# colmap/glomap

Measured on NVIDIA H100. Metric: observations/sec per BA LM-iteration, higher is better.
Workload: dtype f64

## Files before the change

### glomap_b200/csrc/b200sfm.cu

```cuda
#include "../../include/b200sfm.h"

#include <new>

#include "ba_solver.cuh"
#include "context.cuh"
#include "gp_solver.cuh"
#include "ra_solver.cuh"
#include "track_kernels.cuh"

namespace {

cudaStream_t pool_stream(const b200sfm_ctx* ctx) {
  static const bool dist_pool = !(getenv("B200SFM_ASYNC_ALLOC_DIST") && atoi(getenv("B200SFM_ASYNC_ALLOC_DIST")) == 0);
  return ctx && (ctx->world == 1 || dist_pool) ? ctx->stream : nullptr;
}

template <class F>
int guarded(b200sfm_ctx* ctx, F&& f) {
  b200::AllocScope alloc_scope(pool_stream(ctx));
  try {
    return f();
  } catch (const b200::CudaError& e) {
    if (ctx) ctx->err = "CUDA error: " + e.msg + " (line " + std::to_string(e.line) + ")";
    return B200SFM_ERR_CUDA;
// ... 155 lines not shown
void b200sfm_destroy(b200sfm_ctx* ctx) {
  if (!ctx) return;
  cudaSetDevice(ctx->device);
  if (ctx->comm) nccl_api().CommDestroy(ctx->comm);
  if (ctx->p2p.ready) {
    cudaStreamSynchronize(ctx->stream);
    if (ctx->comm) {
      double* d = nullptr;
      if (cudaMalloc(&d, sizeof(double)) == cudaSuccess) {
        cudaMemsetAsync(d, 0, sizeof(double), ctx->stream);
        nccl_api().AllReduce(d, d, 1, ncclFloat64, ncclSum, ctx->comm, ctx->stream);
        cudaStreamSynchronize(ctx->stream);
        cudaFree(d);
      }
    }
    ctx->p2p.release();
  }
  if (ctx->comm_stream) {
    cudaStreamSynchronize(ctx->comm_stream);
    cudaStreamDestroy(ctx->comm_stream);
    cudaEventDestroy(ctx->ev_half);
    cudaEventDestroy(ctx->ev_comm);
  }
  if (ctx->stream) {
    cudaStreamSynchronize(ctx->stream);
    cudaStreamDestroy(ctx->stream);
  }
  if (b200::async_alloc_enabled()) {
    cudaMemPool_t pool;
    if (cudaDeviceGetDefaultMemPool(&pool, ctx->device) == cudaSuccess) cudaMemPoolTrimTo(pool, 0);
    cudaGetLastError();
  }
  if (ctx->h_scal) cudaFreeHost(ctx->h_scal);
  delete ctx;
}

const char* b200sfm_last_error(const b200sfm_ctx* ctx) { return ctx ? ctx->err.c_str() : "null context"; }
int b200sfm_rank(const b200sfm_ctx* ctx) { return ctx ? ctx->rank : -1; }
int b200sfm_world_size(const b200sfm_ctx* ctx) { return ctx ? ctx->world : -1; }
void* b200sfm_cuda_stream(const b200sfm_ctx* ctx) { return ctx ? (void*)ctx->stream : nullptr; }
int64_t b200sfm_kernel_launches(const b200sfm_ctx* ctx) { return ctx ? ctx->launches : 0; }

void b200sfm_ba_default_opts(b200sfm_ba_opts* o) {
  if (!o) return;
  std::memset(o, 0, sizeof(*o));
  o->optimize_rig_poses = 0;
// ... 645 lines not shown
```

### glomap_b200/csrc/ba_kernels_v2.cuh

```cuda
#pragma once
#include "ba_kernels.cuh"
#include "pcg.cuh"

namespace b200 {

struct BAViewV2 {
  const double* Ap;
  double* z4;
  const double* pts4;
  double* Ufk = nullptr;
  const IntrVarRec* ivar = nullptr;
  int C = 0;
};

template <int NK>
__device__ __forceinline__ void obs_intr_rows(const ObsCore& o, const double* __restrict__ ir, const IntrVarRec& iv,
                                              const double Jp[6], double Jk[2][NK > 0 ? NK : 1],
                                              double B[NK > 0 ? 3 * NK : 1]) {
#pragma unroll
  for (int j = 0; j < NK; ++j) {
    double jx = 0.0, jy = 0.0;
    if (j < iv.mb) intr_param_jac(ir, iv.pidx[j], o.uv[0], o.uv[1], 1.0, jx, jy);
    if (!o.valid) jx = jy = 0.0;
    Jk[0][j] = jx;
// ... 473 lines not shown
  a3 = block_sum(a3, scratch);
  if (threadIdx.x == 0) {
    double* o = out + 4 * (size_t)blockIdx.x;
    o[0] = a0; o[1] = a1; o[2] = a2; o[3] = a3;
  }
}

__global__ void ba2_point_rhs_z(BAView v, BAViewV2 v2) {
  const int p = blockIdx.x * blockDim.x + threadIdx.x;
  if (p >= v.P) return;
  double vi[6], g[3], z[3];
#pragma unroll
  for (int k = 0; k < 6; ++k) vi[k] = v.Vinv[6 * (size_t)p + k];
#pragma unroll
  for (int k = 0; k < 3; ++k) g[k] = v.gp[3 * (size_t)p + k];
  sym3_mul(vi, g, z);
  const bool pvalid = (int)(v.pt_begin[p + 1] - v.pt_begin[p]) >= v.min_views;
  *reinterpret_cast<double4*>(v2.z4 + 4 * (size_t)p) = pvalid ? make_double4(z[0], z[1], z[2], 0.0) : make_double4(0, 0, 0, 0);
}

template <int NK>
__global__ void __launch_bounds__(128, B200_PB_MIN_CTAS) ba2_pass_b(BAView v, BAViewV2 v2, const double* __restrict__ cam_rec,
                                                 const double* __restrict__ intr_rec, double huber_a,
                                                 double* __restrict__ y, const PcgCtl* __restrict__ ctl, int seg_lo,
                                                 int seg_hi) {
  if (ctl && ctl->done) return;
  const int warp = seg_lo + ((blockIdx.x * blockDim.x + threadIdx.x) >> 5);
  const int lane = threadIdx.x & 31;
  if (warp >= seg_hi) return;
  const int cam = v.seg_cam[warp];
  const int b = v.seg_begin[warp], e = v.seg_end[warp];
  const double4 q4c = ld_rec32(cam_rec + (size_t)cam * kCamRec);
  const double4 t4c = ld_rec32(cam_rec + (size_t)cam * kCamRec + 4);
  const int blk = v.seg_intr[warp];
  const double* irc = intr_rec + (size_t)blk * kIntrRec;
  const double* src = sensor_of_seg(v, warp);
  constexpr int NKK = NK > 0 ? NK : 1;
  IntrVarRec iv{};
  if (NK > 0) iv = v2.ivar[blk];
  double acc[6] = {0, 0, 0, 0, 0, 0};
  double accK[NKK];
#pragma unroll
  for (int k = 0; k < NKK; ++k) accK[k] = 0.0;
  const uint64_t keep = l2_policy_evict_last();
  int i = b + lane;
  int pt_nxt = 0;
  double4 X = make_double4(0, 0, 0, 0), z = X;
  double2 xy = make_double2(0, 0);
  if (i < e) {
    const int pt0 = ld_stream(v.pt_c + i);
    if (i + 32 < e) pt_nxt = ld_stream(v.pt_c + i + 32);
    X = ld_rec32(v2.pts4 + 4 * (size_t)pt0);
    z = ld_keep4(v2.z4 + 4 * (size_t)pt0, keep);
    xy = ld_stream(v.xy_c + i);
  }
  for (; i < e; i += 32) {
    double4 Xn = X, zn = z;
    double2 xyn = xy;
    int pt_nn = 0;
    if (i + 32 < e) {
      Xn = ld_rec32(v2.pts4 + 4 * (size_t)pt_nxt);
      zn = ld_keep4(v2.z4 + 4 * (size_t)pt_nxt, keep);
      xyn = ld_stream(v.xy_c + i + 32);
    }
    if (i + 64 < e) pt_nn = ld_stream(v.pt_c + i + 64);
    ObsCore o;
    obs_core(q4c, t4c, irc, src, X.x, X.y, X.z, xy, huber_a, o);
    double Jp[6], a[6], bo[3];
    obs_point_blocks(o, Jp, a, bo);
    const double w0 = a[0] * z.x + a[1] * z.y + a[2] * z.z;
    const double w1 = a[1] * z.x + a[3] * z.y + a[4] * z.z;
    const double w2 = a[2] * z.x + a[4] * z.y + a[5] * z.z;
    acc[0] += 2.0 * (X.y * w2 - X.z * w1);
    acc[1] += 2.0 * (X.z * w0 - X.x * w2);
    acc[2] += 2.0 * (X.x * w1 - X.y * w0);
    acc[3] += w0;
    acc[4] += w1;
    acc[5] += w2;
    if (NK > 0) {
      double Jk[2][NKK], Bo[3 * NKK];
      obs_intr_rows<NK>(o, irc, iv, Jp, Jk, Bo);
#pragma unroll
      for (int k = 0; k < NK; ++k) accK[k] += Bo[3 * k] * z.x + Bo[3 * k + 1] * z.y + Bo[3 * k + 2] * z.z;
    }
    X = Xn; z = zn; xy = xyn; pt_nxt = pt_nn;
  }
#pragma unroll
  for (int k = 0; k < 6; ++k) acc[k] = warp_sum(acc[k]);
  if (lane < 6) {
    const int mask = (int)(__double_as_longlong(t4c.w) & 0xff);
    const double q[4] = {q4c.x, q4c.y, q4c.z, q4c.w};
    double R[9];
    quat_to_R(q, R);
    const int bl = lane / 3, r = lane % 3;
    const bool fixed = bl == 0 ? (mask & 1) : (mask & 2);
    const double s = R[3 * r] * acc[3 * bl] + R[3 * r + 1] * acc[3 * bl + 1] + R[3 * r + 2] * acc[3 * bl + 2];
    if (!fixed && s != 0.0) atomicAdd(&y[(size_t)cam * 6 + lane], -s);
  }
  if (NK > 0) {
    const size_t kb = (size_t)(v2.C + blk);
#pragma unroll
    for (int k = 0; k < NK; ++k) {
      const double sk = warp_sum(accK[k]);
      if (lane == 0 && sk != 0.0) atomicAdd(&y[kb * 6 + k], -sk);
    }
  }
}

__global__ void ba2k_pack_xk(int C, const double* __restrict__ cam_rec, const double* __restrict__ x, double* __restrict__ xp,
                             const PcgCtl* __restrict__ ctl) {
  if (ctl && ctl->done) return;
  const int c = blockIdx.x * blockDim.x + threadIdx.x;
  if (c >= C) return;
  const int blk = (int)(__double_as_longlong(cam_rec[(size_t)c * kCamRec + 7]) >> 8);
  xp[(size_t)c * kXqStride + 6] = x[(size_t)(C + blk) * 6];
  xp[(size_t)c * kXqStride + 7] = x[(size_t)(C + blk) * 6 + 1];
}

template <int NK>
__global__ void __launch_bounds__(256) ba2k_cross(int C, int K, const double* __restrict__ cam_rec, const double* __restrict__ Ufk,
                                                  const double* __restrict__ x, double* __restrict__ y,
                                                  const PcgCtl* __restrict__ ctl) {
  constexpr int kBins = 256;
  __shared__ double bins[kBins * NK];
  if (ctl && ctl->done) return;
  const bool use_bins = K <= kBins;
  if (use_bins) {
// ... 42 lines not shown
```

### glomap_b200/csrc/ba_kernels_v3.cuh

```cuda
#pragma once
#include "ba_kernels_v2.cuh"

namespace b200 {

constexpr int kEllWindow = 1024;
constexpr int kEllThreads = 128;

struct EllView {
  int n_groups;
  const int* row0;
  const int* pt;
  const int* len;
  const int* cam;
  const double2* xy;
  const unsigned short* sensor;
  double* A;
  double* B = nullptr;
};

template <class Sort>
__global__ void __launch_bounds__(kEllWindow) ell_sort_window(int P, int min_views, const unsigned* __restrict__ pt_begin,
                                                              int* __restrict__ ell_pt, int* __restrict__ ell_len,
                                                              int* __restrict__ ell_slot, int* __restrict__ group_rows) {
  __shared__ typename Sort::TempStorage tmp;
// ... 241 lines not shown
  if (threadIdx.x == 0) part_cost[blockIdx.x] = cost;
}

__global__ void __launch_bounds__(1024) ba3_reduce_partials(int n, const double* __restrict__ part_a,
                                                           const double* __restrict__ part_b, double* __restrict__ out_sum,
                                                           double* __restrict__ out_max) {
  __shared__ double scratch[32];
  double s = 0.0, m = 0.0;
  for (int i = threadIdx.x; i < n; i += blockDim.x) {
    s += part_a[i];
    if (part_b) m = fmax(m, part_b[i]);
  }
  s = block_sum(s, scratch);
  if (threadIdx.x == 0) *out_sum = s;
  if (part_b) {
    m = block_max(m, scratch);
    if (threadIdx.x == 0) *out_max = m;
  }
}

template <int MODE, int NK>
__global__ void __launch_bounds__(kEllThreads, MODE == 0 ? B200_EA_MIN_CTAS : B200_EA2_MIN_CTAS) ba3_pass_a(
    BAView v, EllView ell, BAViewV2 v2, const double* __restrict__ xp, const double* __restrict__ points,
    double* __restrict__ points_new, double radius, double* __restrict__ bscal, const PcgCtl* __restrict__ ctl) {
  __shared__ double scratch[32];
  if (ctl && ctl->done) return;
  const int slot = blockIdx.x * kEllThreads + threadIdx.x;
  const int lane = threadIdx.x & 31;
  const int g = slot >> 5;
  double b0 = 0, b1 = 0, b2 = 0, b3 = 0;
  if (g < ell.n_groups) {
    const int pt = ell.pt[slot];
    const int mylen = ell.len[slot];
    const int r0 = ell.row0[g], nrow = ell.row0[g + 1] - r0;
    double X0 = 0, X1 = 0, X2 = 0;
    if (pt >= 0) {
      X0 = points[3 * (size_t)pt]; X1 = points[3 * (size_t)pt + 1]; X2 = points[3 * (size_t)pt + 2];
    }
    double s0 = 0, s1 = 0, s2 = 0;
#pragma unroll 4
    for (int j = 0; j < nrow; ++j) {
      if (j >= mylen) continue;
      const size_t idx = ((size_t)r0 + j) * 32 + lane;
      const int cam = ld_stream(ell.cam + idx);
      const double* row = ell.A + ((size_t)r0 + j) * (6 * 32) + lane;
      const double a0 = ld_stream(row), a1 = ld_stream(row + 32), a2 = ld_stream(row + 64);
      const double a3 = ld_stream(row + 96), a4 = ld_stream(row + 128), a5 = ld_stream(row + 160);
      double xr0, xr1, xr2, xt0;
      ld_nc_256(xp + (size_t)cam * kXqStride, xr0, xr1, xr2, xt0);
      double4 xt;
      if (NK > 0) {
        xt = ld_rec32(xp + (size_t)cam * kXqStride + 4);
      } else {
        const double2 xt12 = __ldg(reinterpret_cast<const double2*>(xp + (size_t)cam * kXqStride + 4));
// ... 71 lines not shown
```

### glomap_b200/csrc/ba_solver.cuh

```cuda
#pragma once
#include <cub/cub.cuh>

#include <algorithm>
#include <climits>
#include <cmath>
#include <cstdlib>
#include <vector>

#include "../../include/b200sfm_testing.h"
#include "ba_kernels.cuh"
#include "ba_kernels_v2.cuh"
#include "ba_kernels_v3.cuh"
#include "ba_kernels_ext.cuh"
#include "filter_kernels.cuh"
#include "processor_kernels.cuh"
#include "context.cuh"
#include "pcg.cuh"

namespace b200 {

constexpr double kSliceL2Share = 1.0 / 6.0;

__global__ void k_expand_obs_pt(int P, const unsigned* __restrict__ pt_begin, int* __restrict__ obs_pt) {
  const int p = blockIdx.x * blockDim.x + threadIdx.x;
// ... 79 lines not shown
  if (n > 0) {
    const double inv = 1.0 / n;
    for (int k = 0; k < 4; ++k) q[4 * c + k] *= inv;
  }
}
__global__ void k_rhs(int n, const double* __restrict__ gc, const double* __restrict__ y, double* __restrict__ b) {
  const int i = blockIdx.x * blockDim.x + threadIdx.x;
  if (i < n) b[i] = -(gc[i] + (y ? y[i] : 0.0));
}

}

struct b200sfm_ba_problem {
  using BAView = b200::BAView;
  template <class T>
  using DevBuf = b200::DevBuf<T>;

  b200sfm_ctx* ctx = nullptr;
  int C = 0, P = 0, K = 0;
  long long N = 0;
  int Nv = 0, n_tiles = 0, n_segs = 0, min_views = 3;
  int seg_mid = 0;
  int n_slices = 1, slice_pts = 0;
  long long n_obs_used = 0;

  DevBuf<int> obs_cam, obs_pt, tile_pt_begin, camord_obs, pt_c, seg_cam, seg_begin, seg_end, cam_intr, intr_model;
  int S = 0;
  DevBuf<unsigned short> obs_sensor;
  DevBuf<int> seg_sensor, seg_intr, sensor_intr;
  DevBuf<double> sensor_rec;
  DevBuf<double2> obs_xy, xy_c;
  DevBuf<int4> tile_desc;
  DevBuf<unsigned> pt_begin;
  DevBuf<unsigned char> cam_mask_base, cam_mask;
  DevBuf<double> blk_used;
  DevBuf<double> quat[2], trans[2], points[2], intr, intr_cand, quat_saved, trans_saved, points_saved, intr_saved;
  int CB = 0, nbk = 0;
  bool ext = false, ext_k = false, ext_s = false;
  std::vector<int> h_intr_model;
  std::vector<b200::IntrVarRec> h_ivar;
  DevBuf<b200::IntrVarRec> ivar;
  std::vector<unsigned char> h_sensor_var;
  DevBuf<unsigned char> sensor_var;
  DevBuf<double> sens_q[2], sens_t[2], sens_q_saved, sens_t_saved;
  b200::ExtView ext_view() {
    b200::ExtView e;
// ... 165 lines not shown
                obs_cam.p, S > 0 ? obs_sensor.p : nullptr, obs_pt.p, pt_begin.p, keys.p, vals.p, cam_count.p, bad.p);
    int end_bit = 1;
    while ((1ll << end_bit) <= n_buckets) ++end_bit;
    size_t tmp_bytes = 0;
    cub::DeviceRadixSort::SortPairs(nullptr, tmp_bytes, keys.p, keys_out.p, vals.p, camord_obs.p, (int)N, 0, end_bit, s);
    size_t scan_bytes = 0;
    cub::DeviceScan::ExclusiveSum(nullptr, scan_bytes, cam_count.p, cam_begin.p, n_buckets + 1, s);
    DevBuf<unsigned char> tmp;
    tmp.alloc(std::max(tmp_bytes, scan_bytes) + 16);
    size_t tb = tmp.bytes();
    cub::DeviceRadixSort::SortPairs(tmp.p, tb, keys.p, keys_out.p, vals.p, camord_obs.p, (int)N, 0, end_bit, s);
    ctx->launches += 8;
    tb = tmp.bytes();
    cub::DeviceScan::ExclusiveSum(tmp.p, tb, cam_count.p, cam_begin.p, n_buckets + 1, s);
    B200_LAUNCH(ctx, k_seg_counts, cdiv(n_buckets, 256), 256, 0, n_buckets, cam_count.p, seg_count.p);
    blk_used.alloc(CB);
    blk_used.zero(s);
    B200_LAUNCH(ctx, k_block_used, cdiv(VC, 256), 256, 0, VC, n_groups, smul, C, K, cam_count.p, cam_intr.p,
                S > 0 ? sensor_intr.p : nullptr, blk_used.p);
    ctx->allreduce_sum(blk_used.p, CB);
    tb = tmp.bytes();
    cub::DeviceScan::ExclusiveSum(tmp.p, tb, seg_count.p, seg_off.p, n_buckets + 1, s);
    ctx->launches += 4;
    int h_tot[4];
    B200_CUDA_OK(cudaMemcpyAsync(&h_tot[0], cam_begin.p + n_buckets, sizeof(int), cudaMemcpyDeviceToHost, s));
    B200_CUDA_OK(cudaMemcpyAsync(&h_tot[1], seg_off.p + n_buckets, sizeof(int), cudaMemcpyDeviceToHost, s));
    B200_CUDA_OK(cudaMemcpyAsync(&h_tot[2], bad.p, sizeof(int), cudaMemcpyDeviceToHost, s));
    B200_CUDA_OK(cudaMemcpyAsync(&h_tot[3], seg_off.p + (size_t)n_slices * VC, sizeof(int), cudaMemcpyDeviceToHost, s));
    B200_CUDA_OK(cudaStreamSynchronize(s));
    if (h_tot[2]) throw InvalidInput{"obs_cam out of range [0, C)"};
    Nv = h_tot[0];
    n_segs = h_tot[1];
    seg_mid = h_tot[3];
    seg_cam.alloc(std::max(n_segs, 1)); seg_begin.alloc(std::max(n_segs, 1)); seg_end.alloc(std::max(n_segs, 1));
    seg_sensor.alloc(std::max(n_segs, 1)); seg_intr.alloc(std::max(n_segs, 1));
    pt_c.alloc(std::max(Nv, 1)); xy_c.alloc(std::max(Nv, 1));
    B200_LAUNCH(ctx, k_fill_segs, cdiv(n_buckets, 256), 256, 0, n_buckets, VC, smul, cam_begin.p, seg_off.p, cam_intr.p,
                S > 0 ? sensor_intr.p : nullptr, seg_cam.p, seg_sensor.p, seg_intr.p, seg_begin.p, seg_end.p);
    if (Nv > 0)
      B200_LAUNCH(ctx, k_gather_camorder, cdiv(Nv, 256), 256, 0, Nv, camord_obs.p, obs_pt.p, obs_xy.p, pt_c.p, xy_c.p);

    {
      using Sort = cub::BlockRadixSort<unsigned, kEllWindow, 1, int>;
      const int n_win = cdiv(P, kEllWindow);
      ell_groups = n_win * (kEllWindow / 32);
      ell_ctas = cdiv((long long)ell_groups * 32, kEllThreads);
      ell_pt.alloc((size_t)ell_groups * 32); ell_len.alloc((size_t)ell_groups * 32); ell_slot.alloc(P);
      ell_row0.alloc((size_t)ell_groups + 1);
      DevBuf<int> grows;
      grows.alloc((size_t)ell_groups + 1);
      grows.zero(s);
      B200_LAUNCH(ctx, (ell_sort_window<Sort>), n_win, kEllWindow, 0, P, min_views, pt_begin.p, ell_pt.p, ell_len.p, ell_slot.p, grows.p);
      size_t need = 0;
      cub::DeviceScan::ExclusiveSum(nullptr, need, grows.p, ell_row0.p, ell_groups + 1, s);
      DevBuf<unsigned char> tmp3;
      tmp3.alloc(need + 16);
// ... 324 lines not shown
    ExtView ex = ext_view();
    const int sgrid = cdiv((long long)n_segs * 32, 128);
    if (x && points_var) {
#define B200_EXT_A(WK, WS)                                                                                              \
  B200_LAUNCH(ctx, (bax_pass_a<0, WK, WS>), ell_ctas, kEllThreads, 0, v, ell_view(), ex, view2(), cam_rec.p, intr_rec.p, x, \
              points[cur].p, nullptr, huber_a, radius, nullptr, ctl)
      if (ext_k && ext_s) B200_EXT_A(true, true);
      else if (ext_k) B200_EXT_A(true, false);
      else if (ext_s) B200_EXT_A(false, true);
      else B200_EXT_A(false, false);
#undef B200_EXT_A
    }
    if (n_segs > 0) {
#define B200_EXT_B(WK, WS)                                                                                              \
  B200_LAUNCH(ctx, (bax_pass_b<WK, WS>), sgrid, 128, 0, v, ex, view2(), cam_rec.p, intr_rec.p, points[cur].p, x, huber_a, y, ctl)
      if (ext_k && ext_s) B200_EXT_B(true, true);
      else if (ext_k) B200_EXT_B(true, false);
      else if (ext_s) B200_EXT_B(false, true);
      else B200_EXT_B(false, false);
#undef B200_EXT_B
    }
  }

  void launch_pass_b(const b200::BAView& v, double huber_a, double* y, const b200::PcgCtl* ctl, int seg_lo = 0,
                     int seg_hi = -1) {
    using namespace b200;
    if (seg_hi < 0) seg_hi = n_segs;
    if (seg_hi <= seg_lo) return;
    const int grid = cdiv((long long)(seg_hi - seg_lo) * 32, 128);
#define B200_PASS_B(NKV) \
  B200_LAUNCH(ctx, ba2_pass_b<NKV>, grid, 128, 0, v, view2(), cam_rec.p, intr_rec.p, huber_a, y, ctl, seg_lo, seg_hi)
    if (kfast && nk == 2) B200_PASS_B(2);
    else if (kfast) B200_PASS_B(1);
    else B200_PASS_B(0);
#undef B200_PASS_B
  }
  void launch_pass_a0(const b200::BAView& v, double radius, const b200::PcgCtl* ctl) {
    using namespace b200;
    if (kfast && nk == 2)
      B200_LAUNCH(ctx, (ba3_pass_a<0, 2>), ell_ctas, kEllThreads, 0, v, ell_view(), view2(), xq.p, points[cur].p, nullptr, radius, nullptr, ctl);
    else if (kfast)
      B200_LAUNCH(ctx, (ba3_pass_a<0, 1>), ell_ctas, kEllThreads, 0, v, ell_view(), view2(), xq.p, points[cur].p, nullptr, radius, nullptr, ctl);
    else
      B200_LAUNCH(ctx, (ba3_pass_a<0, 0>), ell_ctas, kEllThreads, 0, v, ell_view(), view2(), xq.p, points[cur].p, nullptr, radius, nullptr, ctl);
  }
  void launch_cross(const double* x, double* y, const b200::PcgCtl* ctl) {
    using namespace b200;
    if (nk == 2) B200_LAUNCH(ctx, ba2k_cross<2>, cdiv(C, 256), 256, 0, C, K, cam_rec.p, Ufk.p, x, y, ctl);
    else B200_LAUNCH(ctx, ba2k_cross<1>, cdiv(C, 256), 256, 0, C, K, cam_rec.p, Ufk.p, x, y, ctl);
  }

  bool matrix_free() const { return ext && !kfast; }
  bool schur_jacobi_on(const b200sfm_ba_opts& o, bool points_var) const {
    return points_var && o.preconditioner == 1 && !matrix_free();
  }

  void matvec(const double* x, double* y, const b200sfm_ba_opts& o, double radius, bool points_var, bool split_ar,
              bool profile, const b200::PcgCtl* ctl) {
    using namespace b200;
    cudaStream_t s = ctx->stream;
    BAView v = view();
    const int nB6 = nbk * 6;
    cudaEvent_t e0 = nullptr, e1 = nullptr;
    if (profile) {
      e0 = timer_mv.next();
      e1 = timer_mv.next();
      B200_CUDA_OK(cudaEventRecord(e0, s));
    }
    if (matrix_free()) {
      ext_matvec(x, y, o.thres_loss_function, radius, points_var, ctl);
    } else if (kfast && !points_var) {
      launch_cross(x, y, ctl);
    } else if (use_v2) {
      if (use_ell)
        launch_pass_a0(v, radius, ctl);
      else
        B200_LAUNCH(ctx, ba2_pass_a<0>, n_tiles, kTile, smem_k3v2, v, view2(), xq.p, points[cur].p, nullptr, radius, nullptr, ctl);
      if (kfast) launch_cross(x, y, ctl);
      if (split_ar) {
        launch_pass_b(v, o.thres_loss_function, y, ctl, 0, seg_mid);
        B200_CUDA_OK(cudaEventRecord(ctx->ev_half, s));
        B200_CUDA_OK(cudaStreamWaitEvent(ctx->comm_stream, ctx->ev_half, 0));
        ctx->allreduce_sum_on(ctx->comm_stream, y, (size_t)(C / 2) * 6);
        B200_CUDA_OK(cudaEventRecord(ctx->ev_comm, ctx->comm_stream));
        launch_pass_b(v, o.thres_loss_function, y, ctl, seg_mid, n_segs);
      } else if (n_segs > 0) {
        launch_pass_b(v, o.thres_loss_function, y, ctl);
      }
    } else {
      B200_LAUNCH(ctx, ba_schur_pass<0>, n_tiles, kTile, smem_k3, v, x, y, nullptr, nullptr, radius, nullptr, nullptr,
                  nullptr, 0, ctl);
    }
    if (profile) B200_CUDA_OK(cudaEventRecord(e1, s));
    if (split_ar) {
      ctx->allreduce_sum(y + (size_t)(C / 2) * 6, nB6 - (size_t)(C / 2) * 6);
      B200_CUDA_OK(cudaStreamWaitEvent(s, ctx->ev_comm, 0));
    } else {
      ctx->allreduce_sum(y, nB6);
    }
  }

  StepResult compute_step(const b200sfm_ba_opts& o, double radius, bool points_var, bool set_jscale_p, bool profile) {
    using namespace b200;
    cudaStream_t s = ctx->stream;
    BAView v = view();
    const int nB6 = nbk * 6;
    if (points_var) B200_LAUNCH(ctx, ba_damp_points, cdiv(P, 256), 256, 0, P, V.p, jscale_p.p, set_jscale_p ? 1 : 0, radius, Vinv.p);
    B200_LAUNCH(ctx, ba_damp_cams, cdiv(nB6, 256), 256, 0, nbk, U(), jscale_c.p, radius, Dc.p);
    const bool recomp = matrix_free();
    const bool schur_jacobi = schur_jacobi_on(o, points_var);
    double* yrhs = Sd.p + (size_t)CB * 21;
    Sd.zero(s);
    if (schur_jacobi && n_segs > 0) {
      if (use_v2)
        B200_LAUNCH(ctx, ba2_schur_diag, cdiv((long long)n_segs * 32, 128), 128, 0, v, view2(), cam_rec.p, intr_rec.p,
                    o.thres_loss_function);
      else B200_LAUNCH(ctx, ba_schur_diag, cdiv((long long)n_segs * 32, 128), 128, 0, v);
    }
    if (points_var) {
      if (use_v2) {
        B200_LAUNCH(ctx, ba2_point_rhs_z, cdiv(P, 256), 256, 0, v, view2());
        if (recomp) ext_matvec(nullptr, yrhs, o.thres_loss_function, radius, true, nullptr);
        else if (n_segs > 0) launch_pass_b(v, o.thres_loss_function, yrhs, nullptr);
      } else {
        B200_LAUNCH(ctx, ba_schur_pass<1>, n_tiles, kTile, smem_k3, v, nullptr, yrhs, nullptr, nullptr, radius, nullptr);
      }
    } else if (recomp) {
      z4.zero(s);
    }
    if (schur_jacobi || points_var) ctx->allreduce_sum(Sd.p, (size_t)CB * 27);
    B200_LAUNCH(ctx, ba_build_precond, cdiv(nbk, 128), 128, 0, nbk, U(), Dc.p, schur_jacobi ? Sd.p : nullptr, Minv.p);
    B200_LAUNCH(ctx, k_rhs, cdiv(nB6, 256), 256, 0, nB6, gc(), points_var ? yrhs : nullptr, bvec.p);
    const int max_it = std::max(1, o.pcg_max_iterations);
    const int nblk = cdiv(nbk, kPcgThreads);
    ctx->pcgh.ensure(max_it, (size_t)nblk * 3, ctx->world);
    double* part_pq = ctx->pcgh.d_part;
    double* part_rz = ctx->pcgh.d_part + nblk;
    double* part_rr = ctx->pcgh.d_part + 2 * (size_t)nblk;
    PcgCtl* ctl = ctx->pcgh.d_ctl;
    StepResult res;
    const size_t mv_ev0 = timer_mv.used;
    const bool has_mv = points_var || ext;
    const bool split_ar = ctx->world > 1 && use_v2 && !recomp && points_var && C >= 64 &&
                          (getenv("B200SFM_SPLIT_AR") && atoi(getenv("B200SFM_SPLIT_AR")) == 1);
    if (split_ar) ctx->ensure_comm_stream();
    const bool pack_dir = points_var && use_v2 && !recomp;
// ... 32 lines not shown
      B200_CUDA_OK(cudaMemcpyAsync(intr_cand.p, intr.p, intr.bytes(), cudaMemcpyDeviceToDevice, s));
      if (S > 0) {
        B200_CUDA_OK(cudaMemcpyAsync(sens_q[nxt].p, sens_q[cur].p, sens_q[cur].bytes(), cudaMemcpyDeviceToDevice, s));
        B200_CUDA_OK(cudaMemcpyAsync(sens_t[nxt].p, sens_t[cur].p, sens_t[cur].bytes(), cudaMemcpyDeviceToDevice, s));
      }
    }
    if (points_var && use_v2) {
      const int nrow_part = use_ell ? ell_ctas : n_tiles;
      if (recomp) {
        ExtView ex = ext_view();
#define B200_EXT_A2(WK, WS)                                                                                                  \
  B200_LAUNCH(ctx, (bax_pass_a<2, WK, WS>), ell_ctas, kEllThreads, 0, v, ell_view(), ex, view2(), cam_rec.p, intr_rec.p, px.p, \
              points[cur].p, points[nxt].p, o.thres_loss_function, radius, bpart.p, nullptr)
        if (ext_k && ext_s) B200_EXT_A2(true, true);
        else if (ext_k) B200_EXT_A2(true, false);
        else if (ext_s) B200_EXT_A2(false, true);
        else B200_EXT_A2(false, false);
#undef B200_EXT_A2
      } else {
        B200_LAUNCH(ctx, ba2_pack_x, cdiv(C, 256), 256, 0, C, px.p, cam_rec.p, xq.p);
        if (kfast) B200_LAUNCH(ctx, ba2k_pack_xk, cdiv(C, 256), 256, 0, C, cam_rec.p, px.p, xq.p, nullptr);
        if (use_ell && kfast && nk == 2)
          B200_LAUNCH(ctx, (ba3_pass_a<2, 2>), ell_ctas, kEllThreads, 0, v, ell_view(), view2(), xq.p, points[cur].p, points[nxt].p, radius,
                      bpart.p, nullptr);
        else if (use_ell && kfast)
          B200_LAUNCH(ctx, (ba3_pass_a<2, 1>), ell_ctas, kEllThreads, 0, v, ell_view(), view2(), xq.p, points[cur].p, points[nxt].p, radius,
                      bpart.p, nullptr);
        else if (use_ell)
          B200_LAUNCH(ctx, (ba3_pass_a<2, 0>), ell_ctas, kEllThreads, 0, v, ell_view(), view2(), xq.p, points[cur].p, points[nxt].p, radius,
                      bpart.p, nullptr);
        else
          B200_LAUNCH(ctx, ba2_pass_a<2>, n_tiles, kTile, smem_k3v2, v, view2(), xq.p, points[cur].p, points[nxt].p, radius, bpart.p, nullptr);
      }
      const int nb = std::min(cdiv(nrow_part, 256), 296);
      B200_LAUNCH(ctx, ba2_sum4_stage1, nb, 256, 0, nrow_part, bpart.p, bpart2.p);
      B200_LAUNCH(ctx, ba_colsum, 4, 256, 0, nb, 4, bpart2.p, scal.p + 2);
    } else if (points_var) {
      B200_LAUNCH(ctx, ba_schur_pass<2>, n_tiles, kTile, smem_k3, v, px.p, nullptr, points[cur].p, points[nxt].p, radius,
                  scal.p + 2);
    } else {
      B200_CUDA_OK(cudaMemcpyAsync(points[nxt].p, points[cur].p, points[cur].bytes(), cudaMemcpyDeviceToDevice, s));
    }
    B200_LAUNCH(ctx, ba_update_cams, cdiv(C, 128), 128, 0, C, quat[cur].p, trans[cur].p, px.p, gc(), pr.p, Dc.p, jscale_c.p,
                blk_used.p, cam_mask.p, quat[nxt].p, trans[nxt].p, scal.p + 8);
    build_records(nxt);
    launch_cost(nxt, o.thres_loss_function);
    ctx->allreduce_sum(scal.p + 2, 11);
    B200_CUDA_OK(cudaMemcpyAsync(ctx->h_scal, scal.p, 16 * sizeof(double), cudaMemcpyDeviceToHost, s));
    B200_CUDA_OK(cudaStreamSynchronize(s));
    double* h = ctx->h_scal;
    for (int k = 8; k <= 12; ++k) h[k] /= (double)ctx->world;
    const double g_dot_d = h[8] + h[2];
    const double dDd = h[10] + h[3];
// ... 225 lines not shown
```

### glomap_b200/csrc/context.cuh

```cuda
#pragma once
#include <dlfcn.h>
#include <nccl.h>

#include <cstring>
#include <string>
#include <vector>

#include "../../include/b200sfm.h"
#include "common.cuh"
#include "p2p_allreduce.cuh"
#include "pcg.cuh"

struct NcclApi {
  void* lib = nullptr;
  ncclResult_t (*GetUniqueId)(ncclUniqueId*) = nullptr;
  ncclResult_t (*CommInitRank)(ncclComm_t*, int, ncclUniqueId, int) = nullptr;
  ncclResult_t (*CommDestroy)(ncclComm_t) = nullptr;
  ncclResult_t (*CommAbort)(ncclComm_t) = nullptr;
  ncclResult_t (*AllReduce)(const void*, void*, size_t, ncclDataType_t, ncclRedOp_t, ncclComm_t, cudaStream_t) = nullptr;
  const char* (*GetErrorString)(ncclResult_t) = nullptr;
  bool load(std::string& err) {
    if (lib) return true;
    lib = dlopen("libnccl.so.2", RTLD_NOW | RTLD_GLOBAL);
    if (!lib) lib = dlopen("libnccl.so", RTLD_NOW | RTLD_GLOBAL);
// ... 41 lines not shown
  void allreduce_sum(double* buf, size_t n) {
    if (world > 1 && p2p.ready && n > 0 && n <= p2p.cap && (reinterpret_cast<uintptr_t>(buf) & 15) == 0) {
      p2p.launch(stream, buf, n);
      ++p2p_calls;
      ++launches;
      return;
    }
    allreduce_sum_on(stream, buf, n);
  }
  void allreduce_sum_on(cudaStream_t st, double* buf, size_t n) {
    if (world == 1 || n == 0) return;
    if (!comm) throw NcclError{"communicator was aborted after an earlier failure"};
    ncclResult_t r = nccl_api().AllReduce(buf, buf, n, ncclFloat64, ncclSum, comm, st);
    if (r != ncclSuccess) throw NcclError{std::string("ncclAllReduce(sum): ") + nccl_api().GetErrorString(r)};
  }
  cudaStream_t comm_stream = nullptr;
  cudaEvent_t ev_half = nullptr, ev_comm = nullptr;
  void ensure_comm_stream() {
    if (comm_stream) return;
    B200_CUDA_OK(cudaStreamCreateWithFlags(&comm_stream, cudaStreamNonBlocking));
    B200_CUDA_OK(cudaEventCreateWithFlags(&ev_half, cudaEventDisableTiming));
    B200_CUDA_OK(cudaEventCreateWithFlags(&ev_comm, cudaEventDisableTiming));
  }
  void allreduce_max(double* buf, size_t n) {
    if (world == 1 || n == 0) return;
    if (!comm) throw NcclError{"communicator was aborted after an earlier failure"};
    ncclResult_t r = nccl_api().AllReduce(buf, buf, n, ncclFloat64, ncclMax, comm, stream);
    if (r != ncclSuccess) throw NcclError{std::string("ncclAllReduce(max): ") + nccl_api().GetErrorString(r)};
  }
};

namespace b200 {

inline cudaStream_t& alloc_stream() {
  static thread_local cudaStream_t s = nullptr;
  return s;
}
struct AllocScope {
  cudaStream_t prev;
  explicit AllocScope(cudaStream_t s) : prev(alloc_stream()) { alloc_stream() = s; }
  ~AllocScope() { alloc_stream() = prev; }
};
inline bool async_alloc_enabled() {
  static const bool on = !(getenv("B200SFM_ASYNC_ALLOC") && atoi(getenv("B200SFM_ASYNC_ALLOC")) == 0);
  return on;
}
// ... 58 lines not shown
  a.accessPolicyWindow.num_bytes = 0;
  cudaStreamSetAttribute(s, cudaStreamAttributeAccessPolicyWindow, &a);
  cudaCtxResetPersistingL2Cache();
  cudaGetLastError();
}

struct EventTimer {
  std::vector<cudaEvent_t> ev;
  size_t used = 0;
  ~EventTimer() {
    for (auto e : ev) cudaEventDestroy(e);
  }
  cudaEvent_t next() {
    if (used == ev.size()) {
      cudaEvent_t e;
      B200_CUDA_OK(cudaEventCreate(&e));
      ev.push_back(e);
    }
    return ev[used++];
  }
  void reset() { used = 0; }
};

#define B200_LAUNCH(ctx, kernel, grid, block, smem, ...)                       \
  do {                                                                         \
    kernel<<<(grid), (block), (smem), (ctx)->stream>>>(__VA_ARGS__);           \
    ++(ctx)->launches;                                                         \
  } while (0)

inline int cdiv(long long a, long long b) { return (int)((a + b - 1) / b); }

}
```

### profiles/kernel_times.py

```python
#!/usr/bin/env python
import argparse
import collections
import os
import sys

ROOT = os.path.dirname(os.path.dirname(os.path.abspath(__file__)))
sys.path.insert(0, ROOT)


def main():
    ap = argparse.ArgumentParser()
    ap.add_argument("--workload", default="config4")
    ap.add_argument("--optimize-intrinsics", type=int, default=0)
    ap.add_argument("--solves", type=int, default=2)
    ap.add_argument("--top", type=int, default=14)
    args = ap.parse_args()
    import torch
    from bench import WORKLOADS
    from glomap_b200 import estimators as E, synthetic as S

    C, P, L, chunk = WORKLOADS[args.workload]
    sc = S.make_scene(C, P, L, seed=1, pixel_sigma=0.5, chunk=chunk, point_range=(0, P))
    init = S.perturb_scene(sc, chunk=chunk, point_offset=0)
    mask = E.first_frame_mask(C)
    torch.cuda.set_device(0)
    ctx = E.Context(0, 0, 1, None)
    opts = E.BundleAdjusterOptions(optimize_intrinsics=bool(args.optimize_intrinsics))
    opts.solver_options.max_num_iterations = 20
    opts.solver_options.pcg_rel_tolerance = 0.05
    opts.solver_options.pcg_max_iterations = 200
    torch.cuda.synchronize()
    free0 = torch.cuda.mem_get_info()[0]
    prob = E.BAProblem(ctx, sc, 3, mask)
    prob.set_state(init.intr_params, init.quat, init.trans, init.points)
    prob.save_state()
    prob.solve(opts)
    torch.cuda.synchronize()
    free1 = torch.cuda.mem_get_info()[0]
    its = []
    with torch.profiler.profile(activities=[torch.profiler.ProfilerActivity.CUDA]) as prof:
        for _ in range(args.solves):
            prob.restore_state()
            st = prob.solve(opts).as_dict()
            its.append((st["iterations"], st["pcg_iterations"]))
        torch.cuda.synchronize()
    agg = collections.defaultdict(lambda: [0, 0.0])
    for ev in prof.events():
        if ev.device_type == torch.autograd.DeviceType.CUDA and ev.name and not ev.name.startswith("Memcpy") \
                and not ev.name.startswith("Memset"):
            name = ev.name.split("(")[0].replace("void ", "").replace("b200::", "")
            agg[name][0] += 1
            agg[name][1] += ev.device_time_total
    tot = sum(v[1] for v in agg.values())
    print(f"{args.workload} optimize_intrinsics={args.optimize_intrinsics} env="
          f"{ {k: v for k, v in os.environ.items() if k.startswith('B200SFM_')} } LM/PCG per solve {its}")
    print(f"device memory held by the resident problem after one solve: {(free0 - free1) / 1e9:.3f} GB")
    print("| kernel | launches | total ms | avg us |\n|---|---|---|---|")
    for k, (n, us) in sorted(agg.items(), key=lambda kv: -kv[1][1])[:args.top]:
        print(f"| `{k}` | {n} | {us / 1e3:.3f} | {us / n:.1f} |")
    print(f"total kernel time {tot / 1e3 / args.solves:.2f} ms per solve\n")
    prob.free()
    ctx.close()


if __name__ == "__main__":
    main()
```

Measured before the change: 1.155 billion.

## Pipeline Schur matvec by point slice, overlapping pass A and pass B on two streams

Splits the PCG mat-vec into per-point-slice chunks. Pass A runs on the main stream for each slice, and the matching pass B camera segments run on a high-priority second stream, gated by per-slice events, so the two passes overlap instead of running back to back. Both kernels become grid-stride loops over segment ranges with capped grid sizes, and the setup code copies per-slice segment offsets to the host. This adds more launches, event traffic and an extra stream, and it relies on the segment ordering matching the point slices.

```diff
diff --git a/glomap_b200/csrc/b200sfm.cu b/glomap_b200/csrc/b200sfm.cu
--- a/glomap_b200/csrc/b200sfm.cu
+++ b/glomap_b200/csrc/b200sfm.cu
@@ -201,6 +201,11 @@
     cudaEventDestroy(ctx->ev_half);
     cudaEventDestroy(ctx->ev_comm);
   }
+  if (ctx->mv_stream) {
+    cudaStreamSynchronize(ctx->mv_stream);
+    cudaStreamDestroy(ctx->mv_stream);
+  }
+  for (cudaEvent_t e : ctx->mv_ev) cudaEventDestroy(e);
   if (ctx->stream) {
     cudaStreamSynchronize(ctx->stream);
     cudaStreamDestroy(ctx->stream);
diff --git a/glomap_b200/csrc/ba_kernels_v2.cuh b/glomap_b200/csrc/ba_kernels_v2.cuh
--- a/glomap_b200/csrc/ba_kernels_v2.cuh
+++ b/glomap_b200/csrc/ba_kernels_v2.cuh
@@ -519,87 +519,89 @@
 template <int NK>
 __global__ void __launch_bounds__(128, B200_PB_MIN_CTAS) ba2_pass_b(BAView v, BAViewV2 v2, const double* __restrict__ cam_rec,
                                                  const double* __restrict__ intr_rec, double huber_a,
-                                                 double* __restrict__ y, const PcgCtl* __restrict__ ctl, int seg_lo,
-                                                 int seg_hi) {
+                                                 double* __restrict__ y, const PcgCtl* __restrict__ ctl, int lo0,
+                                                 int hi0, int lo1, int hi1) {
   if (ctl && ctl->done) return;
-  const int warp = seg_lo + ((blockIdx.x * blockDim.x + threadIdx.x) >> 5);
   const int lane = threadIdx.x & 31;
-  if (warp >= seg_hi) return;
-  const int cam = v.seg_cam[warp];
-  const int b = v.seg_begin[warp], e = v.seg_end[warp];
-  const double4 q4c = ld_rec32(cam_rec + (size_t)cam * kCamRec);
-  const double4 t4c = ld_rec32(cam_rec + (size_t)cam * kCamRec + 4);
-  const int blk = v.seg_intr[warp];
-  const double* irc = intr_rec + (size_t)blk * kIntrRec;
-  const double* src = sensor_of_seg(v, warp);
-  constexpr int NKK = NK > 0 ? NK : 1;
-  IntrVarRec iv{};
-  if (NK > 0) iv = v2.ivar[blk];
-  double acc[6] = {0, 0, 0, 0, 0, 0};
-  double accK[NKK];
-#pragma unroll
-  for (int k = 0; k < NKK; ++k) accK[k] = 0.0;
-  const uint64_t keep = l2_policy_evict_last();
-  int i = b + lane;
-  int pt_nxt = 0;
-  double4 X = make_double4(0, 0, 0, 0), z = X;
-  double2 xy = make_double2(0, 0);
-  if (i < e) {
-    const int pt0 = ld_stream(v.pt_c + i);
-    if (i + 32 < e) pt_nxt = ld_stream(v.pt_c + i + 32);
-    X = ld_rec32(v2.pts4 + 4 * (size_t)pt0);
-    z = ld_keep4(v2.z4 + 4 * (size_t)pt0, keep);
-    xy = ld_stream(v.xy_c + i);
-  }
-  for (; i < e; i += 32) {
-    double4 Xn = X, zn = z;
-    double2 xyn = xy;
-    int pt_nn = 0;
-    if (i + 32 < e) {
-      Xn = ld_rec32(v2.pts4 + 4 * (size_t)pt_nxt);
-      zn = ld_keep4(v2.z4 + 4 * (size_t)pt_nxt, keep);
-      xyn = ld_stream(v.xy_c + i + 32);
-    }
-    if (i + 64 < e) pt_nn = ld_stream(v.pt_c + i + 64);
-    ObsCore o;
-    obs_core(q4c, t4c, irc, src, X.x, X.y, X.z, xy, huber_a, o);
-    double Jp[6], a[6], bo[3];
-    obs_point_blocks(o, Jp, a, bo);
-    const double w0 = a[0] * z.x + a[1] * z.y + a[2] * z.z;
-    const double w1 = a[1] * z.x + a[3] * z.y + a[4] * z.z;
-    const double w2 = a[2] * z.x + a[4] * z.y + a[5] * z.z;
-    acc[0] += 2.0 * (X.y * w2 - X.z * w1);
-    acc[1] += 2.0 * (X.z * w0 - X.x * w2);
-    acc[2] += 2.0 * (X.x * w1 - X.y * w0);
-    acc[3] += w0;
-    acc[4] += w1;
-    acc[5] += w2;
+  const int n0 = hi0 - lo0, n = n0 + (hi1 - lo1);
+  for (int w = (blockIdx.x * blockDim.x + threadIdx.x) >> 5; w < n; w += (gridDim.x * blockDim.x) >> 5) {
+    const int warp = w < n0 ? lo0 + w : lo1 + (w - n0);
+    const int cam = v.seg_cam[warp];
+    const int b = v.seg_begin[warp], e = v.seg_end[warp];
+    const double4 q4c = ld_rec32(cam_rec + (size_t)cam * kCamRec);
+    const double4 t4c = ld_rec32(cam_rec + (size_t)cam * kCamRec + 4);
+    const int blk = v.seg_intr[warp];
+    const double* irc = intr_rec + (size_t)blk * kIntrRec;
+    const double* src = sensor_of_seg(v, warp);
+    constexpr int NKK = NK > 0 ? NK : 1;
+    IntrVarRec iv{};
+    if (NK > 0) iv = v2.ivar[blk];
+    double acc[6] = {0, 0, 0, 0, 0, 0};
+    double accK[NKK];
+  #pragma unroll
+    for (int k = 0; k < NKK; ++k) accK[k] = 0.0;
+    const uint64_t keep = l2_policy_evict_last();
+    int i = b + lane;
+    int pt_nxt = 0;
+    double4 X = make_double4(0, 0, 0, 0), z = X;
+    double2 xy = make_double2(0, 0);
+    if (i < e) {
+      const int pt0 = ld_stream(v.pt_c + i);
+      if (i + 32 < e) pt_nxt = ld_stream(v.pt_c + i + 32);
+      X = ld_rec32(v2.pts4 + 4 * (size_t)pt0);
+      z = ld_keep4(v2.z4 + 4 * (size_t)pt0, keep);
+      xy = ld_stream(v.xy_c + i);
+    }
+    for (; i < e; i += 32) {
+      double4 Xn = X, zn = z;
+      double2 xyn = xy;
+      int pt_nn = 0;
+      if (i + 32 < e) {
+        Xn = ld_rec32(v2.pts4 + 4 * (size_t)pt_nxt);
+        zn = ld_keep4(v2.z4 + 4 * (size_t)pt_nxt, keep);
+        xyn = ld_stream(v.xy_c + i + 32);
+      }
+      if (i + 64 < e) pt_nn = ld_stream(v.pt_c + i + 64);
+      ObsCore o;
+      obs_core(q4c, t4c, irc, src, X.x, X.y, X.z, xy, huber_a, o);
+      double Jp[6], a[6], bo[3];
+      obs_point_blocks(o, Jp, a, bo);
+      const double w0 = a[0] * z.x + a[1] * z.y + a[2] * z.z;
+      const double w1 = a[1] * z.x + a[3] * z.y + a[4] * z.z;
+      const double w2 = a[2] * z.x + a[4] * z.y + a[5] * z.z;
+      acc[0] += 2.0 * (X.y * w2 - X.z * w1);
+      acc[1] += 2.0 * (X.z * w0 - X.x * w2);
+      acc[2] += 2.0 * (X.x * w1 - X.y * w0);
+      acc[3] += w0;
+      acc[4] += w1;
+      acc[5] += w2;
+      if (NK > 0) {
+        double Jk[2][NKK], Bo[3 * NKK];
+        obs_intr_rows<NK>(o, irc, iv, Jp, Jk, Bo);
+  #pragma unroll
+        for (int k = 0; k < NK; ++k) accK[k] += Bo[3 * k] * z.x + Bo[3 * k + 1] * z.y + Bo[3 * k + 2] * z.z;
+      }
+      X = Xn; z = zn; xy = xyn; pt_nxt = pt_nn;
+    }
+  #pragma unroll
+    for (int k = 0; k < 6; ++k) acc[k] = warp_sum(acc[k]);
+    if (lane < 6) {
+      const int mask = (int)(__double_as_longlong(t4c.w) & 0xff);
+      const double q[4] = {q4c.x, q4c.y, q4c.z, q4c.w};
+      double R[9];
+      quat_to_R(q, R);
+      const int bl = lane / 3, r = lane % 3;
+      const bool fixed = bl == 0 ? (mask & 1) : (mask & 2);
+      const double s = R[3 * r] * acc[3 * bl] + R[3 * r + 1] * acc[3 * bl + 1] + R[3 * r + 2] * acc[3 * bl + 2];
+      if (!fixed && s != 0.0) atomicAdd(&y[(size_t)cam * 6 + lane], -s);
+    }
     if (NK > 0) {
-      double Jk[2][NKK], Bo[3 * NKK];
-      obs_intr_rows<NK>(o, irc, iv, Jp, Jk, Bo);
-#pragma unroll
-      for (int k = 0; k < NK; ++k) accK[k] += Bo[3 * k] * z.x + Bo[3 * k + 1] * z.y + Bo[3 * k + 2] * z.z;
-    }
-    X = Xn; z = zn; xy = xyn; pt_nxt = pt_nn;
-  }
-#pragma unroll
-  for (int k = 0; k < 6; ++k) acc[k] = warp_sum(acc[k]);
-  if (lane < 6) {
-    const int mask = (int)(__double_as_longlong(t4c.w) & 0xff);
-    const double q[4] = {q4c.x, q4c.y, q4c.z, q4c.w};
-    double R[9];
-    quat_to_R(q, R);
-    const int bl = lane / 3, r = lane % 3;
-    const bool fixed = bl == 0 ? (mask & 1) : (mask & 2);
-    const double s = R[3 * r] * acc[3 * bl] + R[3 * r + 1] * acc[3 * bl + 1] + R[3 * r + 2] * acc[3 * bl + 2];
-    if (!fixed && s != 0.0) atomicAdd(&y[(size_t)cam * 6 + lane], -s);
-  }
-  if (NK > 0) {
-    const size_t kb = (size_t)(v2.C + blk);
-#pragma unroll
-    for (int k = 0; k < NK; ++k) {
-      const double sk = warp_sum(accK[k]);
-      if (lane == 0 && sk != 0.0) atomicAdd(&y[kb * 6 + k], -sk);
+      const size_t kb = (size_t)(v2.C + blk);
+  #pragma unroll
+      for (int k = 0; k < NK; ++k) {
+        const double sk = warp_sum(accK[k]);
+        if (lane == 0 && sk != 0.0) atomicAdd(&y[kb * 6 + k], -sk);
+      }
     }
   }
 }
diff --git a/glomap_b200/csrc/ba_kernels_v3.cuh b/glomap_b200/csrc/ba_kernels_v3.cuh
--- a/glomap_b200/csrc/ba_kernels_v3.cuh
+++ b/glomap_b200/csrc/ba_kernels_v3.cuh
@@ -287,14 +287,14 @@
 template <int MODE, int NK>
 __global__ void __launch_bounds__(kEllThreads, MODE == 0 ? B200_EA_MIN_CTAS : B200_EA2_MIN_CTAS) ba3_pass_a(
     BAView v, EllView ell, BAViewV2 v2, const double* __restrict__ xp, const double* __restrict__ points,
-    double* __restrict__ points_new, double radius, double* __restrict__ bscal, const PcgCtl* __restrict__ ctl) {
+    double* __restrict__ points_new, double radius, double* __restrict__ bscal, const PcgCtl* __restrict__ ctl,
+    int g_lo, int g_hi) {
   __shared__ double scratch[32];
   if (ctl && ctl->done) return;
-  const int slot = blockIdx.x * kEllThreads + threadIdx.x;
   const int lane = threadIdx.x & 31;
-  const int g = slot >> 5;
   double b0 = 0, b1 = 0, b2 = 0, b3 = 0;
-  if (g < ell.n_groups) {
+  for (int g = g_lo + ((blockIdx.x * kEllThreads + threadIdx.x) >> 5); g < g_hi; g += gridDim.x * (kEllThreads / 32)) {
+    const int slot = g * 32 + lane;
     const int pt = ell.pt[slot];
     const int mylen = ell.len[slot];
     const int r0 = ell.row0[g], nrow = ell.row0[g + 1] - r0;
diff --git a/glomap_b200/csrc/ba_solver.cuh b/glomap_b200/csrc/ba_solver.cuh
--- a/glomap_b200/csrc/ba_solver.cuh
+++ b/glomap_b200/csrc/ba_solver.cuh
@@ -125,6 +125,7 @@
   int Nv = 0, n_tiles = 0, n_segs = 0, min_views = 3;
   int seg_mid = 0;
   int n_slices = 1, slice_pts = 0;
+  std::vector<int> slice_seg;
   long long n_obs_used = 0;
 
   DevBuf<int> obs_cam, obs_pt, tile_pt_begin, camord_obs, pt_c, seg_cam, seg_begin, seg_end, cam_intr, intr_model;
@@ -336,16 +337,17 @@
     tb = tmp.bytes();
     cub::DeviceScan::ExclusiveSum(tmp.p, tb, seg_count.p, seg_off.p, n_buckets + 1, s);
     ctx->launches += 4;
-    int h_tot[4];
+    int h_tot[2];
     B200_CUDA_OK(cudaMemcpyAsync(&h_tot[0], cam_begin.p + n_buckets, sizeof(int), cudaMemcpyDeviceToHost, s));
-    B200_CUDA_OK(cudaMemcpyAsync(&h_tot[1], seg_off.p + n_buckets, sizeof(int), cudaMemcpyDeviceToHost, s));
-    B200_CUDA_OK(cudaMemcpyAsync(&h_tot[2], bad.p, sizeof(int), cudaMemcpyDeviceToHost, s));
-    B200_CUDA_OK(cudaMemcpyAsync(&h_tot[3], seg_off.p + (size_t)n_slices * VC, sizeof(int), cudaMemcpyDeviceToHost, s));
+    B200_CUDA_OK(cudaMemcpyAsync(&h_tot[1], bad.p, sizeof(int), cudaMemcpyDeviceToHost, s));
+    slice_seg.assign((size_t)n_groups + 1, 0);
+    B200_CUDA_OK(cudaMemcpy2DAsync(slice_seg.data(), sizeof(int), seg_off.p, (size_t)VC * sizeof(int), sizeof(int),
+                                   (size_t)n_groups + 1, cudaMemcpyDeviceToHost, s));
     B200_CUDA_OK(cudaStreamSynchronize(s));
-    if (h_tot[2]) throw InvalidInput{"obs_cam out of range [0, C)"};
+    if (h_tot[1]) throw InvalidInput{"obs_cam out of range [0, C)"};
     Nv = h_tot[0];
-    n_segs = h_tot[1];
-    seg_mid = h_tot[3];
+    n_segs = slice_seg[n_groups];
+    seg_mid = slice_seg[n_slices];
     seg_cam.alloc(std::max(n_segs, 1)); seg_begin.alloc(std::max(n_segs, 1)); seg_end.alloc(std::max(n_segs, 1));
     seg_sensor.alloc(std::max(n_segs, 1)); seg_intr.alloc(std::max(n_segs, 1));
     pt_c.alloc(std::max(Nv, 1)); xy_c.alloc(std::max(Nv, 1));
@@ -716,27 +718,31 @@
     }
   }
 
-  void launch_pass_b(const b200::BAView& v, double huber_a, double* y, const b200::PcgCtl* ctl, int seg_lo = 0,
-                     int seg_hi = -1) {
-    using namespace b200;
-    if (seg_hi < 0) seg_hi = n_segs;
-    if (seg_hi <= seg_lo) return;
-    const int grid = cdiv((long long)(seg_hi - seg_lo) * 32, 128);
+  void launch_pass_b(cudaStream_t st, const b200::BAView& v, double huber_a, double* y, const b200::PcgCtl* ctl, int lo0,
+                     int hi0, int lo1 = 0, int hi1 = 0, int max_ctas = 0) {
+    using namespace b200;
+    const long long nseg = (long long)(hi0 - lo0) + (hi1 - lo1);
+    if (nseg <= 0) return;
+    int grid = cdiv(nseg * 32, 128);
+    if (max_ctas > 0) grid = std::min(grid, max_ctas);
 #define B200_PASS_B(NKV) \
-  B200_LAUNCH(ctx, ba2_pass_b<NKV>, grid, 128, 0, v, view2(), cam_rec.p, intr_rec.p, huber_a, y, ctl, seg_lo, seg_hi)
+  B200_LAUNCH_ON(ctx, st, ba2_pass_b<NKV>, grid, 128, 0, v, view2(), cam_rec.p, intr_rec.p, huber_a, y, ctl, lo0, hi0, lo1, hi1)
     if (kfast && nk == 2) B200_PASS_B(2);
     else if (kfast) B200_PASS_B(1);
     else B200_PASS_B(0);
 #undef B200_PASS_B
   }
-  void launch_pass_a0(const b200::BAView& v, double radius, const b200::PcgCtl* ctl) {
-    using namespace b200;
-    if (kfast && nk == 2)
-      B200_LAUNCH(ctx, (ba3_pass_a<0, 2>), ell_ctas, kEllThreads, 0, v, ell_view(), view2(), xq.p, points[cur].p, nullptr, radius, nullptr, ctl);
-    else if (kfast)
-      B200_LAUNCH(ctx, (ba3_pass_a<0, 1>), ell_ctas, kEllThreads, 0, v, ell_view(), view2(), xq.p, points[cur].p, nullptr, radius, nullptr, ctl);
-    else
-      B200_LAUNCH(ctx, (ba3_pass_a<0, 0>), ell_ctas, kEllThreads, 0, v, ell_view(), view2(), xq.p, points[cur].p, nullptr, radius, nullptr, ctl);
+  void launch_pass_a0(const b200::BAView& v, double radius, const b200::PcgCtl* ctl, int g_lo, int g_hi, int max_ctas = 0) {
+    using namespace b200;
+    if (g_hi <= g_lo) return;
+    int grid = cdiv((long long)(g_hi - g_lo) * 32, kEllThreads);
+    if (max_ctas > 0) grid = std::min(grid, max_ctas);
+#define B200_PASS_A0(NKV) \
+  B200_LAUNCH(ctx, (ba3_pass_a<0, NKV>), grid, kEllThreads, 0, v, ell_view(), view2(), xq.p, points[cur].p, nullptr, radius, nullptr, ctl, g_lo, g_hi)
+    if (kfast && nk == 2) B200_PASS_A0(2);
+    else if (kfast) B200_PASS_A0(1);
+    else B200_PASS_A0(0);
+#undef B200_PASS_A0
   }
   void launch_cross(const double* x, double* y, const b200::PcgCtl* ctl) {
     using namespace b200;
@@ -747,6 +753,30 @@
   bool matrix_free() const { return ext && !kfast; }
   bool schur_jacobi_on(const b200sfm_ba_opts& o, bool points_var) const {
     return points_var && o.preconditioner == 1 && !matrix_free();
+  }
+
+  bool matvec_overlap_on(bool points_var, bool split_ar) const {
+    return points_var && use_v2 && use_ell && !matrix_free() && !split_ar && n_slices > 1 && n_segs > 0 &&
+           !(getenv("B200SFM_MV_OVERLAP") && atoi(getenv("B200SFM_MV_OVERLAP")) == 0);
+  }
+  void matvec_pipelined(const b200::BAView& v, const double* x, double* y, double huber_a, double radius,
+                        const b200::PcgCtl* ctl) {
+    using namespace b200;
+    cudaStream_t s = ctx->stream;
+    ctx->ensure_mv_stream((size_t)n_slices + 1);
+    cudaStream_t sb = ctx->mv_stream;
+    if (kfast) launch_cross(x, y, ctl);
+    const int gps = slice_pts / 32;
+    const int a_ctas = B200_EA_MIN_CTAS * ctx->num_sms, b_ctas = B200_PB_MIN_CTAS * ctx->num_sms;
+    for (int sl = 0; sl < n_slices; ++sl) {
+      launch_pass_a0(v, radius, ctl, sl * gps, std::min(ell_groups, (sl + 1) * gps), a_ctas);
+      B200_CUDA_OK(cudaEventRecord(ctx->mv_ev[sl], s));
+      B200_CUDA_OK(cudaStreamWaitEvent(sb, ctx->mv_ev[sl], 0));
+      launch_pass_b(sb, v, huber_a, y, ctl, slice_seg[sl], slice_seg[sl + 1], slice_seg[n_slices + sl],
+                    slice_seg[n_slices + sl + 1], b_ctas);
+    }
+    B200_CUDA_OK(cudaEventRecord(ctx->mv_ev[n_slices], sb));
+    B200_CUDA_OK(cudaStreamWaitEvent(s, ctx->mv_ev[n_slices], 0));
   }
 
   void matvec(const double* x, double* y, const b200sfm_ba_opts& o, double radius, bool points_var, bool split_ar,
@@ -765,21 +795,23 @@
       ext_matvec(x, y, o.thres_loss_function, radius, points_var, ctl);
     } else if (kfast && !points_var) {
       launch_cross(x, y, ctl);
+    } else if (matvec_overlap_on(points_var, split_ar)) {
+      matvec_pipelined(v, x, y, o.thres_loss_function, radius, ctl);
     } else if (use_v2) {
       if (use_ell)
-        launch_pass_a0(v, radius, ctl);
+        launch_pass_a0(v, radius, ctl, 0, ell_groups);
       else
         B200_LAUNCH(ctx, ba2_pass_a<0>, n_tiles, kTile, smem_k3v2, v, view2(), xq.p, points[cur].p, nullptr, radius, nullptr, ctl);
       if (kfast) launch_cross(x, y, ctl);
       if (split_ar) {
-        launch_pass_b(v, o.thres_loss_function, y, ctl, 0, seg_mid);
+        launch_pass_b(s, v, o.thres_loss_function, y, ctl, 0, seg_mid);
         B200_CUDA_OK(cudaEventRecord(ctx->ev_half, s));
         B200_CUDA_OK(cudaStreamWaitEvent(ctx->comm_stream, ctx->ev_half, 0));
         ctx->allreduce_sum_on(ctx->comm_stream, y, (size_t)(C / 2) * 6);
         B200_CUDA_OK(cudaEventRecord(ctx->ev_comm, ctx->comm_stream));
-        launch_pass_b(v, o.thres_loss_function, y, ctl, seg_mid, n_segs);
-      } else if (n_segs > 0) {
-        launch_pass_b(v, o.thres_loss_function, y, ctl);
+        launch_pass_b(s, v, o.thres_loss_function, y, ctl, seg_mid, n_segs);
+      } else {
+        launch_pass_b(s, v, o.thres_loss_function, y, ctl, 0, n_segs);
       }
     } else {
       B200_LAUNCH(ctx, ba_schur_pass<0>, n_tiles, kTile, smem_k3, v, x, y, nullptr, nullptr, radius, nullptr, nullptr,
@@ -815,7 +847,7 @@
       if (use_v2) {
         B200_LAUNCH(ctx, ba2_point_rhs_z, cdiv(P, 256), 256, 0, v, view2());
         if (recomp) ext_matvec(nullptr, yrhs, o.thres_loss_function, radius, true, nullptr);
-        else if (n_segs > 0) launch_pass_b(v, o.thres_loss_function, yrhs, nullptr);
+        else launch_pass_b(s, v, o.thres_loss_function, yrhs, nullptr, 0, n_segs);
       } else {
         B200_LAUNCH(ctx, ba_schur_pass<1>, n_tiles, kTile, smem_k3, v, nullptr, yrhs, nullptr, nullptr, radius, nullptr);
       }
@@ -894,13 +926,13 @@
         if (kfast) B200_LAUNCH(ctx, ba2k_pack_xk, cdiv(C, 256), 256, 0, C, cam_rec.p, px.p, xq.p, nullptr);
         if (use_ell && kfast && nk == 2)
           B200_LAUNCH(ctx, (ba3_pass_a<2, 2>), ell_ctas, kEllThreads, 0, v, ell_view(), view2(), xq.p, points[cur].p, points[nxt].p, radius,
-                      bpart.p, nullptr);
+                      bpart.p, nullptr, 0, ell_groups);
         else if (use_ell && kfast)
           B200_LAUNCH(ctx, (ba3_pass_a<2, 1>), ell_ctas, kEllThreads, 0, v, ell_view(), view2(), xq.p, points[cur].p, points[nxt].p, radius,
-                      bpart.p, nullptr);
+                      bpart.p, nullptr, 0, ell_groups);
         else if (use_ell)
           B200_LAUNCH(ctx, (ba3_pass_a<2, 0>), ell_ctas, kEllThreads, 0, v, ell_view(), view2(), xq.p, points[cur].p, points[nxt].p, radius,
-                      bpart.p, nullptr);
+                      bpart.p, nullptr, 0, ell_groups);
         else
           B200_LAUNCH(ctx, ba2_pass_a<2>, n_tiles, kTile, smem_k3v2, v, view2(), xq.p, points[cur].p, points[nxt].p, radius, bpart.p, nullptr);
       }
diff --git a/glomap_b200/csrc/context.cuh b/glomap_b200/csrc/context.cuh
--- a/glomap_b200/csrc/context.cuh
+++ b/glomap_b200/csrc/context.cuh
@@ -87,6 +87,20 @@
     B200_CUDA_OK(cudaEventCreateWithFlags(&ev_half, cudaEventDisableTiming));
     B200_CUDA_OK(cudaEventCreateWithFlags(&ev_comm, cudaEventDisableTiming));
   }
+  cudaStream_t mv_stream = nullptr;
+  std::vector<cudaEvent_t> mv_ev;
+  void ensure_mv_stream(size_t n_events) {
+    if (!mv_stream) {
+      int least = 0, greatest = 0;
+      B200_CUDA_OK(cudaDeviceGetStreamPriorityRange(&least, &greatest));
+      B200_CUDA_OK(cudaStreamCreateWithPriority(&mv_stream, cudaStreamNonBlocking, greatest));
+    }
+    while (mv_ev.size() < n_events) {
+      cudaEvent_t e;
+      B200_CUDA_OK(cudaEventCreateWithFlags(&e, cudaEventDisableTiming));
+      mv_ev.push_back(e);
+    }
+  }
   void allreduce_max(double* buf, size_t n) {
     if (world == 1 || n == 0) return;
     if (!comm) throw NcclError{"communicator was aborted after an earlier failure"};
@@ -191,11 +205,13 @@
   void reset() { used = 0; }
 };
 
-#define B200_LAUNCH(ctx, kernel, grid, block, smem, ...)                       \
+#define B200_LAUNCH_ON(ctx, st, kernel, grid, block, smem, ...)                \
   do {                                                                         \
-    kernel<<<(grid), (block), (smem), (ctx)->stream>>>(__VA_ARGS__);           \
+    kernel<<<(grid), (block), (smem), (st)>>>(__VA_ARGS__);                    \
     ++(ctx)->launches;                                                         \
   } while (0)
+#define B200_LAUNCH(ctx, kernel, grid, block, smem, ...) \
+  B200_LAUNCH_ON(ctx, (ctx)->stream, kernel, grid, block, smem, __VA_ARGS__)
 
 inline int cdiv(long long a, long long b) { return (int)((a + b - 1) / b); }
 
diff --git a/profiles/kernel_times.py b/profiles/kernel_times.py
--- a/profiles/kernel_times.py
+++ b/profiles/kernel_times.py
@@ -25,7 +25,7 @@
     mask = E.first_frame_mask(C)
     torch.cuda.set_device(0)
     ctx = E.Context(0, 0, 1, None)
-    opts = E.BundleAdjusterOptions(optimize_intrinsics=bool(args.optimize_intrinsics))
+    opts = E.BundleAdjusterOptions(optimize_intrinsics=bool(args.optimize_intrinsics), profile_kernels=True)
     opts.solver_options.max_num_iterations = 20
     opts.solver_options.pcg_rel_tolerance = 0.05
     opts.solver_options.pcg_max_iterations = 200
@@ -37,12 +37,13 @@
     prob.solve(opts)
     torch.cuda.synchronize()
     free1 = torch.cuda.mem_get_info()[0]
-    its = []
+    its, mv = [], []
     with torch.profiler.profile(activities=[torch.profiler.ProfilerActivity.CUDA]) as prof:
         for _ in range(args.solves):
             prob.restore_state()
             st = prob.solve(opts).as_dict()
             its.append((st["iterations"], st["pcg_iterations"]))
+            mv.append((st["n_matvec"], st["ms_matvec"]))
         torch.cuda.synchronize()
     agg = collections.defaultdict(lambda: [0, 0.0])
     for ev in prof.events():
@@ -54,6 +55,8 @@
     tot = sum(v[1] for v in agg.values())
     print(f"{args.workload} optimize_intrinsics={args.optimize_intrinsics} env="
           f"{ {k: v for k, v in os.environ.items() if k.startswith('B200SFM_')} } LM/PCG per solve {its}")
+    n_mv, ms_mv = sum(n for n, _ in mv), sum(ms for _, ms in mv)
+    print(f"mat-vec (the solver's CUDA events around all of its kernels): {n_mv} timed, {1e3 * ms_mv / max(n_mv, 1):.1f} us each")
     print(f"device memory held by the resident problem after one solve: {(free0 - free1) / 1e9:.3f} GB")
     print("| kernel | launches | total ms | avg us |\n|---|---|---|---|")
     for k, (n, us) in sorted(agg.items(), key=lambda kv: -kv[1][1])[:args.top]:
```

Measured after the change: 1.168 billion, median of 6. 1.01x the previous value.
